# ethz-asl/multipoint

Measured on AMD Instinct MI355X. Metric: image-pairs/sec (detect+desc+match) @ 480x640, higher is better.
Workload: dtype f32

## Files before the change

multipoint_amd/csrc/api.hip:

```cpp
#include "host.h"

using namespace mp_host;

namespace {

bool debug_switch(const char* key, int* value = nullptr, int dflt = 1)
{
    const char* e = getenv("MP_DEBUG");
    if (!e) return false;
    const size_t kl = std::strlen(key);
    for (const char* q = e; *q;) {
        while (*q == ',' || *q == ' ') ++q;
        const char* end = q;
        while (*end && *end != ',') ++end;
        if ((size_t)(end - q) >= kl && std::strncmp(q, key, kl) == 0 && (q[kl] == '=' || q + kl == end || q[kl] == ' ')) {
            if (value) *value = q[kl] == '=' ? atoi(q + kl + 1) : dflt;
            return true;
        }
        q = end;
    }
    return false;
}

int kfd_num_xcc(const char* bus_id)
// ... 7 lines not shown
        FILE* f = fopen(path, "r");
        if (!f) { if (node > 8) break; else continue; }
        char key[64]; unsigned long long val = 0, loc = ~0ull, domain = 0, xcc = 0, simd = 0;
        while (fscanf(f, "%63s %llu", key, &val) == 2) {
            if (!strcmp(key, "location_id")) loc = val;
            else if (!strcmp(key, "domain")) domain = val;
            else if (!strcmp(key, "num_xcc")) xcc = val;
            else if (!strcmp(key, "simd_count")) simd = val;
        }
        fclose(f);
        if (simd > 0 && loc == want && domain == dom) return (int)xcc;
    }
    return 0;
}

}

extern "C" {

const char* mp_version(void) { return "multipoint_hip 0.1 (gfx950)"; }

const char* mp_last_error(const mp_handle* h) { return h ? h->err.c_str() : g_create_error.c_str(); }

int mp_device_shape(const mp_handle* h, int* compute_units, int* xcds, int* persistent_workgroups)
{
    if (!h) return MP_EINVAL;
    if (compute_units) *compute_units = h->ncu;
    if (xcds) *xcds = 1 << h->xcd_shift;
    if (persistent_workgroups) *persistent_workgroups = (int)persistent_grid(1ll << 40, h->ncu, h->xcd_shift);
    return MP_OK;
}

int mp_create(mp_handle** out, int device)
{
    mp_handle* h = nullptr;
    if (!out) return fail(h, MP_EINVAL, "mp_create: out is NULL");
    *out = nullptr;
    int ndev = 0;
    MP_HIP(hipGetDeviceCount(&ndev));
    if (device < 0 || device >= ndev)
        return fail(h, MP_EINVAL, "mp_create: device " + std::to_string(device) + " not available (" +
                                      std::to_string(ndev) + " HIP devices visible)");
    MP_HIP(hipSetDevice(device));
    {
        static const char* const legacy[] = {"MP_NO_WINOGRAD", "MP_WINO43", "MP_WINO43_GEN", "MP_NO_FUSE", "MP_NO_FUSE43", "MP_NO_HEAD_FUSE",
            "MP_NO_PLANAR", "MP_PLANAR", "MP_NO_PERSIST", "MP_PERSIST_MIN_ITEMS", "MP_SPLITK_MAX", "MP_F16_NO_RES", "MP_F16_NO_FUSE1",
            "MP_F16_RES_GROUPS", "MP_NCU", "MP_NXCD", "MP_POST_OVERLAP", "MP_NO_VIN", "MP_NO_POOL_FIRST"};
        static bool warned = false;
        for (const char* k : legacy)
            if (!warned && getenv(k)) {
                warned = true;
                fprintf(stderr, "libmultipoint_hip: the environment variable %s is no longer read (nor are the other MP_* kernel switches): "
                                "use MP_DEBUG=key[=value],... -- the keys are listed in csrc/api.hip (debug_switch)\n", k);
            }
    }
    hipDeviceProp_t prop;
    MP_HIP(hipGetDeviceProperties(&prop, device));
    if (std::strncmp(prop.gcnArchName, "gfx950", 6) != 0)
        return fail(h, MP_EINVAL, std::string("mp_create: kernels are built for gfx950 only, device is ") +
                                      prop.gcnArchName);
    int ncu = prop.multiProcessorCount, nxcd = 0;
    {
        char bus[64] = {0};
        if (hipDeviceGetPCIBusId(bus, sizeof bus, device) == hipSuccess) nxcd = kfd_num_xcc(bus);
        if (nxcd <= 0) nxcd = ncu >= 32 ? ncu / 32 : 1;
        int v = 0;
        if (debug_switch("ncu", &v) && v > 0 && v <= ncu) ncu = v;
        if (debug_switch("nxcd", &v) && v > 0) nxcd = v;
    }
    if (ncu < 1 || nxcd < 1 || (nxcd & (nxcd - 1)) != 0 || nxcd > ncu)
        return fail(h, MP_EINVAL, "mp_create: unsupported machine shape: " + std::to_string(ncu) + " compute units in " +
                                      std::to_string(nxcd) + " XCDs (the XCD count must be a power of two <= the CU count)");
    int xcd_shift = 0;
    while ((1 << xcd_shift) < nxcd) ++xcd_shift;
    DebugSwitches d;
    int v = 0;
    d.winograd = !debug_switch("no_winograd");
    if (debug_switch("wino43", &v) && v == 0) d.wino43 = false;
    if (debug_switch("wino43_gen", &v) && v >= 0 && v <= 2) d.wino43_gen = v;
    d.fuse_first = !debug_switch("no_fuse");
    d.fuse43 = !debug_switch("no_fuse43");
    d.head_fuse = !debug_switch("no_head_fuse");
    d.vin = !debug_switch("no_vin");
    d.planar = !debug_switch("no_planar");
    d.xplanar = d.planar && !debug_switch("no_xplanar");
    if (debug_switch("persist_min_items", &v) && v > 0) d.persist = v;
    if (debug_switch("no_persist")) d.persist = 0;
    if (debug_switch("splitk_max", &v) && v >= 1 && v <= 8) d.splitk_max = v;
    d.f16_res = !debug_switch("f16_no_res");
    d.f16_fuse1 = !debug_switch("f16_no_fuse1");
    if (debug_switch("f16_res_groups", &v) && v == 2) d.f16_res_groups = 2;
    mp_handle* hh = new mp_handle(device, ncu, xcd_shift, d);
    if (hipHostMalloc(reinterpret_cast<void**>(&hh->pinned), 4096) != hipSuccess) {
        delete hh;
        return fail(h, MP_ENOMEM, "mp_create: hipHostMalloc failed");
    }
    *out = hh;
    return MP_OK;
}

void mp_destroy(mp_handle* h)
{
    if (!h) return;
    (void)hipSetDevice(h->device);
    int* pinned = h->pinned;
    const std::vector<ProfEntry> events = std::move(h->prof_entries);
    delete h;
    if (pinned) (void)hipHostFree(pinned);
    for (auto& e : events) { (void)hipEventDestroy(e.a); (void)hipEventDestroy(e.b); }
}

int mp_profile_enable(mp_handle* h, int enable)
{
    if (!h) return MP_EINVAL;
    h->prof = enable != 0;
    h->prof_used = 0;
    return MP_OK;
}

int mp_profile_read(mp_handle* h, const char** names, float* ms, double* flop, int capacity, int* n)
{
    if (!h || !n) return MP_EINVAL;
    *n = 0;
    for (size_t i = 0; i < h->prof_used && (int)i < capacity; ++i) {
        ProfEntry& e = h->prof_entries[i];
        MP_HIP(hipEventSynchronize(e.b));
        float t = 0.f;
        MP_HIP(hipEventElapsedTime(&t, e.a, e.b));
        if (names) names[i] = e.name;
        if (ms) ms[i] = t;
        if (flop) flop[i] = e.flop;
        ++*n;
    }
    h->prof_used = 0;
    return MP_OK;
}

}
```

multipoint_amd/csrc/conv_wino43.hip:

```cpp
#include "mp_common.h"
#include "mp_device.h"
#include "mp_tile.h"

#include <algorithm>
#include <type_traits>

MP_TIMING_TABLE(g_timing_q, 256 * 8, mp_debug_read_timing_wino43)
MP_TIMING_HEIGHT(g_timing_q_sel, 480, mp_debug_select_height_wino43)

namespace {

constexpr int NPIX = 18 * 34;
constexpr int UC4 = 4;
constexpr int VB4 = UC4 * 32 * 36;
constexpr int UB4 = UC4 * 64 * 36;
constexpr int NRB = (NPIX + 63) / 64;
constexpr int RB4 = NRB * 64 * 4;
constexpr int SW4 = 8 * 36 * 2;


template <int LEAD = 0>
__device__ __forceinline__ void dma16(const float* sbase, unsigned voff_bytes, unsigned lds_byte)
{
    lds_dma<4, LEAD, 0>(sbase, voff_bytes, lds_byte);
}

template <bool POOL, bool BNF, int TC4, bool F1, bool SPLIT = false, bool VIN = false>
__global__ __launch_bounds__(512, 2) void conv_wino43_kernel(const ConvParams p)
{
    static_assert(!(F1 && SPLIT), "the fused first block is never split");
    static_assert(!(VIN && (F1 || SPLIT)), "pre-transformed input: plain launches only");
    constexpr int TR4 = 32 / TC4;
    constexpr int OY = 4 * TR4, OX = 4 * TC4;
    constexpr int PY = OY + 2, PX = OX + 2;
    static_assert(PY * PX == NPIX, "item shape");
    __shared__ __attribute__((aligned(16))) float Vs[(VIN ? 4 : 2) * VB4];
    __shared__ __attribute__((aligned(16))) float Us[2 * UB4];
    __shared__ __attribute__((aligned(16))) float raw[VIN ? 256 : 3 * RB4 + 256];
    __shared__ __attribute__((aligned(16))) float scr[VIN ? 4 : 8 * SW4];
    __shared__ __attribute__((aligned(16))) float prm[(POOL && !SPLIT ? 6 : 3) * 64];

    const int tid = threadIdx.x;
    const int lane = tid & 63;
    const int wave = __builtin_amdgcn_readfirstlane(tid >> 6);
    const int tb = wave & 1, cb = wave >> 1;
    const int NC = SPLIT ? (p.cin / UC4) >> p.ks_shift : p.cin / UC4;

    const XcdRange xr = xcd_range(p.nitems, p.xcd_shift);
    const int stride = xr.stride, item_end = xr.item_end;
    int item = xr.item;
    if (item >= item_end) return;

    struct Where { int slice, img, y0, x0, tile; const float* in_base; };
    auto decode = [&](int it) __attribute__((always_inline)) -> Where {
        Where w{};
        const int tile = (int)udiv((unsigned)it, p.magic_slices, (unsigned)p.nslices);
        w.slice = it - tile * p.nslices;
        w.tile = tile;
        const int trow = (int)udiv((unsigned)tile, p.magic_tx, (unsigned)p.tiles_x);
        const int tx = tile - trow * p.tiles_x;
        const int bi = (int)udiv((unsigned)trow, p.magic_ty, (unsigned)p.tiles_y);
        const int ty = trow - bi * p.tiles_y;
        w.img = p.img_list ? p.img_list[bi] : bi;
        w.y0 = ty * OY; w.x0 = tx * OX;
        w.in_base = p.in_planar ? p.in + (long long)w.img * (p.cin / 4) * p.H * p.W * 4
                                : p.in + (long long)w.img * p.H * p.W * p.in_cstride + p.in_coff;
        if constexpr (SPLIT)
            w.in_base += (long long)((w.slice & ((1 << p.ks_shift) - 1)) * NC) * (p.in_planar ? (long long)p.H * p.W * 4 : UC4);
        return w;
    };

    const int pix_stride = p.in_planar ? 4 : p.in_cstride;
    const long long unit_stride = p.in_planar ? (long long)p.H * p.W * 4 : UC4;
    const int x_shift = p.in_planar == MP_LAYOUT_XPLANAR ? 2 : 0, x_mask = p.in_planar == MP_LAYOUT_XPLANAR ? 3 : 0;
    const int row_stride = p.W * pix_stride;
    auto pixel_off = [&](int y, int x) __attribute__((always_inline)) -> int {
        return y * row_stride + (x >> x_shift) * pix_stride + (x & x_mask) * p.W;
    };
    unsigned rvoff[2];
    bool roff_rel = false;
    auto raw_offsets = [&](const Where& w) __attribute__((always_inline)) -> const float* {
        const bool interior = (w.y0 >= 1) && (w.y0 + OY < p.H) && (w.x0 >= 1) && (w.x0 + OX < p.W);
        if (interior) {
            if (!roff_rel) {
#pragma unroll
                for (int j = 0; j < 2; ++j) {
                    const int f = (wave + 8 * j) * 64 + lane;
                    const int py = f / PX, px = f - py * PX;
                    rvoff[j] = (f < NPIX) ? (unsigned)pixel_off(py, px + x_mask) * 4u : 0u;
                }
                roff_rel = true;
            }
            return w.in_base + pixel_off(w.y0 - 1, w.x0 - 1 - x_mask);
        }
        roff_rel = false;
#pragma unroll
        for (int j = 0; j < 2; ++j) {
            const int f = (wave + 8 * j) * 64 + lane;
            const int py = f / PX, px = f - py * PX;
            unsigned off = 0;
            if (f < NPIX) {
                const int gy = reflect_clamp(w.y0 + py - 1, p.H), gx = reflect_clamp(w.x0 + px - 1, p.W);
                off = (unsigned)pixel_off(gy, gx) * 4u;
            }
            rvoff[j] = off;
        }
        return w.in_base;
    };
    const unsigned raw_lds = lds_addr(raw), us_lds = lds_addr(Us);
    const unsigned raw_m0 = raw_lds + (unsigned)wave * 1024u;
    const unsigned raw_dummy = raw_lds + 3u * RB4 * 4u;
    auto raw_dma = [&](const float* src, unsigned boff_bytes, int j) __attribute__((always_inline)) {
        const unsigned dst = j == 0 ? raw_m0 + boff_bytes : (wave + 8 < NRB ? raw_m0 + 8192u + boff_bytes : raw_dummy);
        dma16(src, rvoff[j], dst);
    };
    const int u_cnt = wave < 4 ? 5 : 4, u_first = wave < 4 ? 5 * wave : 20 + 4 * (wave - 4);
    auto u_dma_site = [&](const float* ub, int buf, int site) __attribute__((always_inline)) {
        if constexpr (VIN) {
#pragma unroll
            for (int i = 3 * site; i < (site ? 5 : 3); ++i) {
                int b = wave + 8 * i;
                b = b < 36 ? b : 35;
                dma16(ub + b * 256, (unsigned)lane * 16u, us_lds + (unsigned)(buf * UB4 + b * 256) * 4u);
            }
            return;
        }
#pragma unroll
        for (int k = 3 * site; k < 3 * site + 3; ++k)
            if (k < u_cnt) {
                const int b = u_first + k;
                dma16<1>(ub + b * 256, (unsigned)lane * 16u, us_lds + (unsigned)(buf * UB4 + b * 256) * 4u);
            }
    };
    auto u_ptr = [&](int slice) __attribute__((always_inline)) -> const float* {
        return p.wpack + (long long)slice * NC * UB4;
    };
    auto load_prm = [&](int vslice) __attribute__((always_inline)) {
        const int slice = SPLIT ? vslice >> p.ks_shift : vslice;
        if (tid < 64) {
            int t = tid;
            if constexpr (F1) asm volatile("" : "+v"(t));
// ... 327 lines not shown
                    acc[s] = __builtin_amdgcn_mfma_f32_16x16x4f32(af[g % 3][e], bf[g % 3][e], FIRST ? zero4 : acc[s], 0, 0, 0);
                    __builtin_amdgcn_sched_barrier(0);
                    if constexpr (!VIN) { if (e != 2) tf_at(g, e, vb); }
                    if constexpr (F1) prod_at(g, e, vb);
                    if (e == 0) {
                        af[(g + 2) % 3] = *reinterpret_cast<const f32x4*>(g + 2 < 9 ? &ur[4 * (g + 2)] : &urn[4 * (g - 7)]);
                        bf[(g + 2) % 3] = *reinterpret_cast<const f32x4*>(g + 2 < 9 ? &vr[4 * (g + 2)] : &vrn[4 * (g - 7)]);
                    } else if (e == 1) {
                        if (g == 7) u_dma_site(un2, vb, 0);
                        else if (g == 8) u_dma_site(un2, vb, 1);
                        else if (g == 0) { if constexpr (VIN) v_dma(vcur, (vs + 3) & 3, 0); else if constexpr (!F1) raw_dma(rsrc, rd_byte, 0); }
                        else if (g == 1) { if constexpr (VIN) v_dma(vcur, (vs + 3) & 3, 1); else if constexpr (!F1) raw_dma(rsrc, rd_byte, 1); }
                        else if (g == 2) { if constexpr (VIN) v_dma(vcur, (vs + 3) & 3, 2); }
                    } else if (e == 2) {
                        if constexpr (!VIN) tf_at(g, 2, vb);
                    } else {
                        if (g == 6) {
#ifdef MP_TIMING
                            t_b0 = __builtin_amdgcn_s_memtime();
#endif
                            if constexpr (F1) asm volatile("s_waitcnt vmcnt(0) lgkmcnt(0)" ::: "memory");
                            else if constexpr (VIN) asm volatile("s_waitcnt vmcnt(3) lgkmcnt(0)" ::: "memory");
                            else asm volatile("s_waitcnt vmcnt(2) lgkmcnt(0)" ::: "memory");
#ifdef MP_TIMING
                            t_b1 = __builtin_amdgcn_s_memtime();
#endif
                            __syncthreads();
#ifdef MP_TIMING
                            tsum[4] += __builtin_amdgcn_s_memtime() - t_b1;
#endif
                        }
                    }
                    __builtin_amdgcn_sched_barrier(0);
                }
            }
            MP_CLOCK(t_u1);
            MP_CLOCK_ADD(0, t_u0, t_u1);
            MP_CLOCK_ADD(1, t_b0, t_b1);
        };
        auto unit = [&](const int c, auto first_tag, auto vb_tag, auto vs_tag) __attribute__((always_inline)) {
            unit_body(c, first_tag, vb_tag, vs_tag);
            if constexpr (VIN) {
                v_advance();
            } else if constexpr (F1) {
                prod_advance();
            } else {
                ld_advance();
                const unsigned ro = 3u * RB4 * 4u - rd_byte - rt_byte;
                rd_byte = rt_byte; rt_byte = ro;
            }
        };
        using VB0 = std::integral_constant<int, 0>;
        using VB1 = std::integral_constant<int, 1>;
        using VS2 = std::integral_constant<int, 2>;
        using VS3 = std::integral_constant<int, 3>;
        if constexpr (VIN) {
            unit(0, std::true_type{}, VB0{}, VB0{});
            for (int c = 1; c + 3 < NC; c += 4) {
                unit(c, std::false_type{}, VB1{}, VB1{});
                unit(c + 1, std::false_type{}, VB0{}, VS2{});
                unit(c + 2, std::false_type{}, VB1{}, VS3{});
                unit(c + 3, std::false_type{}, VB0{}, VB0{});
            }
            unit(NC - 3, std::false_type{}, VB1{}, VB1{});
            unit(NC - 2, std::false_type{}, VB0{}, VS2{});
            unit(NC - 1, std::false_type{}, VB1{}, VS3{});
        } else {
        unit(0, std::true_type{}, VB0{}, VB0{});
        for (int c = 1; c + 1 < NC; c += 2) {
            unit(c, std::false_type{}, VB1{}, VB1{});
            unit(c + 1, std::false_type{}, VB0{}, VB0{});
        }
        unit(NC - 1, std::false_type{}, VB1{}, VB1{});
        }

        MP_CLOCK(t_e0);
        MP_CLOCK_ADD(3, t_item, t_e0);
        if constexpr (F1) { if (item_next + stride < item_end) patch_dma(decode(item_next + stride), cur_par); }
        const int tl = tb * 16 + (lane & 15);
        const int cl = cb * 16 + 4 * (lane >> 4);
        const f32x4 b4 = *reinterpret_cast<const f32x4*>(&prm[cl]);
        const f32x4 s4 = *reinterpret_cast<const f32x4*>(&prm[64 + cl]);
        const f32x4 t4 = *reinterpret_cast<const f32x4*>(&prm[128 + cl]);
        const int oy = cur.y0 + 4 * (tl / TC4), ox = cur.x0 + 4 * (tl % TC4);
        const int ch0 = (SPLIT ? cur.slice >> p.ks_shift : cur.slice) * 64 + cl;
        const int cs = p.out_cstride;
        constexpr int NO = POOL ? 2 : 4;
        f32x2 keep[NO][NO];
        if constexpr (SPLIT) {
            unsigned long long* const part = reinterpret_cast<unsigned long long*>(p.split_scratch) + (long long)item * (2 * 16 * 512) + tid;
#pragma unroll
            for (int h = 0; h < 2; ++h) {
                f32x2 tcol[4][6];
#pragma unroll
                for (int j = 0; j < 6; ++j) {
                    f32x2 m[6], y[4];
#pragma unroll
                    for (int i = 0; i < 6; ++i) m[i] = f32x2{acc[6 * i + j][2 * h], acc[6 * i + j][2 * h + 1]};
                    at6s(m, y);
#pragma unroll
                    for (int a = 0; a < 4; ++a) tcol[a][j] = y[a];
                }
#pragma unroll
                for (int a = 0; a < 4; ++a) {
                    f32x2 y[4];
                    at6s(tcol[a], y);
#pragma unroll
                    for (int b = 0; b < 4; ++b)
                        part[(h * 16 + a * 4 + b) * 512] = __builtin_bit_cast(unsigned long long, y[b]);
                }
            }
        }
        if constexpr (!SPLIT) {
#pragma unroll
        for (int h = 0; h < 2; ++h) {
            f32x2 tcol[4][6];
            if constexpr (!SPLIT) {
#pragma unroll
            for (int j = 0; j < 6; ++j) {
                f32x2 m[6], y[4];
#pragma unroll
                for (int i = 0; i < 6; ++i) m[i] = f32x2{acc[6 * i + j][2 * h], acc[6 * i + j][2 * h + 1]};
                at6s(m, y);
#pragma unroll
                for (int a = 0; a < 4; ++a) tcol[a][j] = y[a];
            }
            }
            const f32x2 bb = {b4[2 * h], b4[2 * h + 1]}, ss = {s4[2 * h], s4[2 * h + 1]}, tt = {t4[2 * h], t4[2 * h + 1]};
            f32x2 res[NO][NO];
            if constexpr (POOL) {
                const f32x4 g4 = *reinterpret_cast<const f32x4*>(&prm[192 + cl]);
                const f32x4 lo4 = *reinterpret_cast<const f32x4*>(&prm[256 + cl]), hi4 = *reinterpret_cast<const f32x4*>(&prm[320 + cl]);
                const f32x2 gg = {g4[2 * h], g4[2 * h + 1]};
                const f32x2 gb = bb * gg;
                constexpr float A1 = (float)MP_W43_A, A2 = A1 * A1, A3 = A2 * A1, A4 = A2 * A2;
                const f32x2 gk[5] = {gg, gg * f32x2{A1, A1}, gg * f32x2{A2, A2}, gg * f32x2{A3, A3}, gg * f32x2{A4, A4}};
                f32x2 xv[4][4];
#pragma unroll
                for (int a = 0; a < 4; ++a) {
                    f32x2 y[4];
                    at6s(tcol[a], y);
#pragma unroll
                    for (int b = 0; b < 4; ++b) {
                        const int e = (a == 1 ? 1 : a == 2 ? 2 : 0) + (b == 1 ? 1 : b == 2 ? 2 : 0);
                        xv[a][b] = __builtin_elementwise_fma(y[b], gk[e], gb);
                    }
                }
#pragma unroll
                for (int a = 0; a < NO; ++a)
#pragma unroll
                    for (int b = 0; b < NO; ++b) {
                        f32x2 m;
#pragma unroll
                        for (int r = 0; r < 2; ++r)
                            m[r] = fmaxf(fmaxf(xv[2 * a][2 * b][r], xv[2 * a][2 * b + 1][r]), fmaxf(xv[2 * a + 1][2 * b][r], xv[2 * a + 1][2 * b + 1][r]));
                        if (BNF) {
                            m = __builtin_elementwise_fma(m, ss, tt);
                            m = f32x2{relu_bits(m[0]), relu_bits(m[1])};
                        } else {
#pragma unroll
                            for (int r = 0; r < 2; ++r)
                                asm("v_med3_i32 %0, %1, %2, %3" : "=v"(m[r]) : "v"(m[r]), "v"(lo4[2 * h + r]), "v"(hi4[2 * h + r]));
                            m = __builtin_elementwise_fma(m, ss, tt);
                        }
                        res[a][b] = m;
                    }
            } else {
            f32x2 yv[4][4];
#pragma unroll
            for (int a = 0; a < 4; ++a) {
                f32x2 y[4];
                at6s(tcol[a], y);
#pragma unroll
                for (int b = 0; b < 4; ++b) {
                    f32x2 v = w43_add_bias(y[b], a, b, bb);
                    if (BNF) { v = v * ss + tt; v = f32x2{relu_bits(v[0]), relu_bits(v[1])}; }
                    else { v = f32x2{relu_bits(v[0]), relu_bits(v[1])}; v = v * ss + tt; }
                    yv[a][b] = v;
                }
            }
#pragma unroll
            for (int a = 0; a < NO; ++a)
#pragma unroll
                for (int b = 0; b < NO; ++b) res[a][b] = yv[a][b];
            }
            if (h == 0) {
#pragma unroll
                for (int a = 0; a < NO; ++a)
#pragma unroll
                    for (int b = 0; b < NO; ++b) keep[a][b] = res[a][b];
            } else {
                const int Ho = POOL ? p.H >> 1 : p.H, Wo = POOL ? p.W >> 1 : p.W;
                const int py0 = POOL ? oy >> 1 : oy, px0 = POOL ? ox >> 1 : ox;
                const bool xpl = !POOL && p.out_planar == MP_LAYOUT_XPLANAR;
                char* const img_base = reinterpret_cast<char*>(
                    p.out_planar ? p.out + (long long)cur.img * (p.cout / 4) * Ho * Wo * 4
                                 : p.out + (long long)cur.img * Ho * Wo * cs + p.out_coff);
                const unsigned ps = xpl ? (unsigned)Wo * 4u : p.out_planar ? 16u : (unsigned)cs * 4u;
                const unsigned rs = p.out_planar ? (unsigned)Wo * 16u : (unsigned)Wo * ps;
                const unsigned o0 = xpl ? (unsigned)(((ch0 >> 2) * Ho + py0) * Wo * 4 + px0) * 4u
                                  : p.out_planar ? (unsigned)(((ch0 >> 2) * Ho + py0) * Wo + px0) * 16u
                                                 : (unsigned)((py0 * Wo + px0) * cs + ch0) * 4u;
                if (oy < p.H && ox < p.W && ch0 < p.cout) {
#pragma unroll
                    for (int a = 0; a < NO; ++a)
#pragma unroll
                        for (int b = 0; b < NO; ++b) {
                            const f32x4 v = {keep[a][b][0], keep[a][b][1], res[a][b][0], res[a][b][1]};
                            *reinterpret_cast<f32x4*>(img_base + (o0 + (unsigned)a * rs + (unsigned)b * ps)) = v;
                        }
                }
            }
        }
        }
        MP_CLOCK(t_e1);
        MP_CLOCK_ADD(2, t_e0, t_e1);
#ifdef MP_TIMING
        tsum[7] += 1;
        if (!has_next && tid == 0 && t_on)
            for (int i = 0; i < 8; ++i) g_timing_q[blockIdx.x * 8 + i] = tsum[i];
#endif
        if (!has_next) { dma_wait(); return; }
        if (next_slice != cur.slice) {
            __syncthreads();
            load_prm(next_slice);
        }
        item = item_next;
        cur = decode(item);
        cur_par ^= 1;
        up = unext;
    }
}

template <int TC4>
__global__ __launch_bounds__(256) void wino43_vprod_kernel(const ConvParams p, long long ntb)
{
    constexpr int TR4 = 32 / TC4, OY = 4 * TR4, OX = 4 * TC4;
    __shared__ __attribute__((aligned(16))) float st[19456];
    const int ncp = p.cin >> 1, NC = p.cin / UC4;
    const int TL = 256 / ncp;
    const int RS = TL * 36 + 4;
    const int groups = 32 / TL;
    const int tid = threadIdx.x;
    const int cp = tid % ncp, tlc = tid / ncp;
    const long long tb = (long long)blockIdx.x / groups;
    const int t0 = ((int)((long long)blockIdx.x % groups)) * TL, t = t0 + tlc;
    (void)ntb;
    const int tx = (int)(tb % p.tiles_x);
    const long long trow = tb / p.tiles_x;
    const int ty = (int)(trow % p.tiles_y);
    const int bi = (int)(trow / p.tiles_y);
    const int img = p.img_list ? p.img_list[bi] : bi;
    const int wy = ty * OY + 4 * (t / TC4) - 1, wx = tx * OX + 4 * (t % TC4) - 1;
    const float* const base = p.in + (long long)img * p.H * p.W * p.in_cstride + p.in_coff + 2 * cp;
    int gx[6];
#pragma unroll
    for (int j = 0; j < 6; ++j) gx[j] = reflect_clamp(wx + j, p.W);
    f32x2 r[6][6];
#pragma unroll
    for (int j = 0; j < 6; ++j) {
        f32x2 d[6], o[6];
#pragma unroll
        for (int i = 0; i < 6; ++i)
            d[i] = *reinterpret_cast<const f32x2*>(base + ((long long)reflect_clamp(wy + i, p.H) * p.W + gx[j]) * p.in_cstride);
        bt6(d, o);
#pragma unroll
        for (int i = 0; i < 6; ++i) r[i][j] = o[i];
    }
    float* const dst0 = st + (2 * cp) * RS + tlc * 36;
    float* const dst1 = dst0 + RS;
#pragma unroll
    for (int i = 0; i < 6; i += 2) {
        f32x2 a[6], b[6];
        bt6(r[i], a);
        bt6(r[i + 1], b);
        *reinterpret_cast<f32x4*>(dst0 + 6 * i) = f32x4{a[0][0], a[1][0], a[2][0], a[3][0]};
        *reinterpret_cast<f32x4*>(dst0 + 6 * i + 4) = f32x4{a[4][0], a[5][0], b[0][0], b[1][0]};
        *reinterpret_cast<f32x4*>(dst0 + 6 * i + 8) = f32x4{b[2][0], b[3][0], b[4][0], b[5][0]};
        *reinterpret_cast<f32x4*>(dst1 + 6 * i) = f32x4{a[0][1], a[1][1], a[2][1], a[3][1]};
        *reinterpret_cast<f32x4*>(dst1 + 6 * i + 4) = f32x4{a[4][1], a[5][1], b[0][1], b[1][1]};
        *reinterpret_cast<f32x4*>(dst1 + 6 * i + 8) = f32x4{b[2][1], b[3][1], b[4][1], b[5][1]};
    }
    __syncthreads();
    const int q4 = TL * 9, total4 = p.cin * q4;
    float* const gbase = p.vglobal + (tb * NC * 4 * 32 + t0) * 36;
    for (int i = tid; i < total4; i += 256) {
        const int row = i / q4, w = i - row * q4;
        *reinterpret_cast<f32x4*>(gbase + (long long)row * (32 * 36) + w * 4) = *reinterpret_cast<const f32x4*>(st + row * RS + w * 4);
    }
}

template <bool POOL, int TC4, bool F1 = false, bool SPLIT = false>
int launch_q(const ConvParams& p, hipStream_t s)
{
    constexpr int OY = 4 * (32 / TC4), OX = 4 * TC4;
    ConvParams q = p;
    if (SPLIT) q.nslices = p.nslices << p.ks_shift;
    q.tiles_x = (p.W + OX - 1) / OX; q.tiles_y = (p.H + OY - 1) / OY;
    const long long nitems = (long long)p.B * q.tiles_x * q.tiles_y * q.nslices;
    if (nitems <= 0) return 0;
    if (tile_items(q, nitems)) return 1;
    const unsigned grid = persistent_grid(nitems, p.ncu, p.xcd_shift);
    const ConvParams& pp = q;
    if (p.bn_first) hipLaunchKernelGGL((conv_wino43_kernel<POOL, true, TC4, F1, SPLIT>), dim3(grid), dim3(512), 0, s, pp);
    else hipLaunchKernelGGL((conv_wino43_kernel<POOL, false, TC4, F1, SPLIT>), dim3(grid), dim3(512), 0, s, pp);
    return 0;
}

template <int TC4>
int launch_vin(const ConvParams& p, hipStream_t s)
{
    constexpr int OY = 4 * (32 / TC4), OX = 4 * TC4;
    ConvParams q = p;
    q.tiles_x = (p.W + OX - 1) / OX; q.tiles_y = (p.H + OY - 1) / OY;
    const long long ntb = (long long)p.B * q.tiles_x * q.tiles_y, nitems = ntb * q.nslices;
    if (nitems <= 0) return 0;
    if (tile_items(q, nitems)) return 1;
    const ConvParams& pp = q;
    const int tl = 256 / (p.cin / 2);
    hipLaunchKernelGGL((wino43_vprod_kernel<TC4>), dim3((unsigned)(ntb * (32 / tl))), dim3(256), 0, s, pp, ntb);
    const unsigned grid = persistent_grid(nitems, p.ncu, p.xcd_shift);
    if (p.bn_first) hipLaunchKernelGGL((conv_wino43_kernel<false, true, TC4, false, false, true>), dim3(grid), dim3(512), 0, s, pp);
    else hipLaunchKernelGGL((conv_wino43_kernel<false, false, TC4, false, false, true>), dim3(grid), dim3(512), 0, s, pp);
    return 0;
}

template <bool POOL, bool SPLIT = false>
int launch_shape(const ConvParams& p, hipStream_t s)
{
    const long long wide = (long long)((p.W + 31) / 32) * ((p.H + 15) / 16), tall = (long long)((p.W + 15) / 16) * ((p.H + 31) / 32);
    return tall < wide ? launch_q<POOL, 4, false, SPLIT>(p, s) : launch_q<POOL, 8, false, SPLIT>(p, s);
}

}

bool conv_wino43_supports(const ConvParams& p)
{
    return !p.pad_zero && p.cin % 8 == 0 && p.cout % 4 == 0 && p.H % 4 == 0 && p.W % 4 == 0 && p.H >= 4 && p.W >= 4 &&
           p.in_cstride % 4 == 0 && p.in_coff % 4 == 0 && p.out_cstride % 4 == 0 && p.out_coff % 4 == 0;
}

long long conv_wino43_vglobal_floats(const ConvParams& p)
{
    const long long wide = (long long)((p.W + 31) / 32) * ((p.H + 15) / 16), tall = (long long)((p.W + 15) / 16) * ((p.H + 31) / 32);
    return (long long)p.B * std::min(wide, tall) * (p.cin / UC4) * VB4;
}

long long conv_wino43_items(const ConvParams& p)
{
    const long long wide = (long long)((p.W + 31) / 32) * ((p.H + 15) / 16), tall = (long long)((p.W + 15) / 16) * ((p.H + 31) / 32);
    return (long long)p.B * std::min(wide, tall) * p.nslices;
}

int launch_conv_wino43(const ConvParams& p, bool pool, hipStream_t s, bool fuse_first)
{
    if (p.out_planar == MP_LAYOUT_XPLANAR && pool) return 2;
    if ((p.in_planar == MP_LAYOUT_XPLANAR || p.out_planar == MP_LAYOUT_XPLANAR) && p.ks_shift > 0) return 2;
    if (fuse_first) return pool && p.cin == 64 ? launch_q<true, 8, true>(p, s) : 2;
    if (p.vglobal) {
        if (pool || p.ks_shift > 0 || p.cin % 16 != 0 || p.in_planar || p.cin > 256 || 256 % (p.cin / 2) != 0 || (p.cin / 2) < 8) return 2;
        const long long wide = (long long)((p.W + 31) / 32) * ((p.H + 15) / 16), tall = (long long)((p.W + 15) / 16) * ((p.H + 31) / 32);
        return tall < wide ? launch_vin<4>(p, s) : launch_vin<8>(p, s);
    }
    if (p.ks_shift > 0) {
        const int ncs = (p.cin / 4) >> p.ks_shift;
        if (ncs < 4 || (ncs & 1) || (ncs << p.ks_shift) * 4 != p.cin || !p.split_scratch) return 2;
        const int rc = pool ? launch_shape<true, true>(p, s) : launch_shape<false, true>(p, s);
        return rc ? rc : launch_split_reduce(p, 1, pool, s);
    }
    return pool ? launch_shape<true>(p, s) : launch_shape<false>(p, s);
}
```

multipoint_amd/csrc/forward.hip:

```cpp
#include "host.h"

using namespace mp_host;

namespace {

int pick_mbw(int H, int W)
{
    long long best = -1;
    int arg = 32;
    for (int mbw : {32, 16, 8}) {
        const int tw = mbw, th = 256 / mbw;
        const long long area = (long long)((H + th - 1) / th) * th * ((W + tw - 1) / tw) * tw;
        if (best < 0 || area < best) { best = area; arg = mbw; }
    }
    return arg;
}

void prof_begin(mp_handle* h, const char* name, double flop, hipStream_t s)
{
    if (!h->prof) return;
    if (h->prof_used == h->prof_entries.size()) {
        ProfEntry e{};
        (void)hipEventCreate(&e.a); (void)hipEventCreate(&e.b);
        h->prof_entries.push_back(e);
// ... 76 lines not shown
    EncoderPlan P;
    if (h->cfg.mixed_precision) {
        const ConvLayer& L0 = E.conv[0];
        P.conv[0].fuse_first = h->dbg.f16_res && h->dbg.f16_fuse1 && h->cfg.reflection_pad && !E.first_pool && L0.pool &&
                               L0.cin == 64 && L0.cout == 64 && L0.nslices == 1;
        for (int i = 0; i < E.nconv; ++i) P.conv[i].kernel = f16_kind(h, E.conv[i], E.conv[i].cin, 0, P.conv[i].fuse_first);
        return P;
    }
    for (int i = 0, hh = E.first_pool ? H / 2 : H, ww = E.first_pool ? W / 2 : W; i < E.nconv; ++i) {
        const ConvLayer& L = E.conv[i];
        ConvLaunch& c = P.conv[i];
        c.kernel = wino43_kind(h, L, hh, ww, L.cin, 0, L.cout, 0);
        if (i == 0) {
            const bool fuse43 = c.kernel == Kernel::wino43 && h->dbg.fuse43 && L.pool && L.cin == 64 && L.cout == 64 &&
                                h->cfg.channel_version == 0 && L.u43pack_f1;
            c.fuse_first = h->dbg.fuse_first && h->cfg.channel_version == 0 && !E.first_pool && (h->policy.direct || fuse43);
        }
        const bool producer = i == 0 ? !E.first_pool : P.conv[i - 1].kernel != Kernel::direct && E.conv[i - 1].pool;
        c.in_planar = h->dbg.planar && c.kernel != Kernel::direct && producer ? MP_LAYOUT_PLANAR : MP_LAYOUT_NHWC;
        plan_split_vin(h, L, nb, hh, ww, fwd_batch, c);
        if (i > 0 && h->dbg.xplanar && !E.conv[i - 1].pool && P.conv[i - 1].kernel == Kernel::wino43 && P.conv[i - 1].ks_shift == 0 &&
            c.kernel == Kernel::wino43 && c.ks_shift == 0 && !c.vin)
            c.in_planar = MP_LAYOUT_XPLANAR;
        if (i > 0) P.conv[i - 1].out_planar = c.in_planar;
        if (L.pool) { hh /= 2; ww /= 2; }
    }
    return P;
}


template <typename P, typename T>
int conv_geometry(const mp_handle* h, const ConvLayer& L, P& p, const T* in, int in_cstride, int in_coff, T* out, int out_cstride,
                  int out_coff, int B, int H, int W)
{
    p.in = in; p.out = out; p.B = B; p.H = H; p.W = W;
    p.in_cstride = in_cstride; p.in_coff = in_coff; p.cin = L.cin;
    p.out_cstride = out_cstride; p.out_coff = out_coff; p.cout = L.cout; p.nslices = L.nslices;
    p.pad_zero = h->cfg.reflection_pad ? 0 : 1; p.bn_first = h->cfg.bn_first;
    p.ncu = h->ncu; p.xcd_shift = h->xcd_shift;
    const int mbw = L.taps == 9 ? pick_mbw(H, W) : 32, th = 256 / mbw;
    if (L.taps == 9) { p.tiles_x = (W + mbw - 1) / mbw; p.tiles_y = (H + th - 1) / th; }
    else p.total_px = (long long)B * H * W;
    return mbw;
}

template <typename P, typename T>
void conv1_geometry(const mp_handle* h, P& c1, const float* images, T* out, int B, int H, int W)
{
    c1.in = images; c1.out = out; c1.B = B; c1.H = H; c1.W = W;
    c1.pad_zero = h->cfg.reflection_pad ? 0 : 1; c1.bn_first = h->cfg.bn_first;
}

template <typename T>
int run_conv(mp_handle* h, const ConvLayer& L, const ConvLaunch& c, const T* in, int in_cstride, int in_coff, T* out,
             int out_cstride, int out_coff, int B, int H, int W, const int* img_list, hipStream_t s,
             const FirstLayer* first = nullptr, const float* images = nullptr)
{
    constexpr bool f16 = std::is_same<T, _Float16>::value;
    typename std::conditional<f16, ConvParamsH, ConvParams>::type p{};
    const int mbw = conv_geometry(h, L, p, in, in_cstride, in_coff, out, out_cstride, out_coff, B, H, W);
    p.scale = L.scale; p.shift = L.shift; p.img_list = img_list;
    if (c.fuse_first) {
        p.img = images; p.w1 = f16 ? first->w_h : first->w; p.b1 = f16 ? first->bias_h : first->bias;
        p.s1 = first->scale; p.t1 = first->shift;
    }
    if constexpr (f16) {
        p.wpack = L.wpack_h; p.bias = L.bias_h;
        p.dummy = static_cast<_Float16*>(h->f16_dummy.p);
        p.res_groups = h->dbg.f16_res_groups;
    } else {
        p.wpack = c.kernel == Kernel::direct ? L.wpack : L.u43pack; p.bias = L.bias;
        p.relu = L.relu ? 1 : 0;
        p.persist = h->dbg.persist;
        p.in_planar = c.in_planar; p.out_planar = c.out_planar;
        if (c.fuse_first && c.kernel != Kernel::direct) {
            p.wpack = L.u43pack_f1; p.bias = L.bias_f1; p.w1 = first->w_f1; p.b1 = first->bias_f1; p.s1 = nullptr; p.t1 = nullptr;
        }
        if (c.ks_shift) {
            const int rc = ensure(h, h->split_ws, (size_t)(conv_wino43_items(p) << c.ks_shift) * (2 * 16 * 512 * 8));
            if (rc) return rc;
            p.ks_shift = c.ks_shift; p.split_scratch = static_cast<float*>(h->split_ws.p);
        }
        if (c.vin) {
            if (ensure(h, h->vin_ws, (size_t)conv_wino43_vglobal_floats(p) * 4) == MP_OK) p.vglobal = static_cast<float*>(h->vin_ws.p);
            else { (void)hipGetLastError(); h->err.clear(); }
        }
    }
    prof_begin(h, c.fuse_first ? "enc.conv1+2" : L.name,
               2.0 * L.taps * L.cin * L.cout * (double)B * H * W + (c.fuse_first ? 2.0 * 9 * 64 * (double)B * H * W : 0.0), s);
    int big = 0;
    if constexpr (f16) {
        if (c.kernel == Kernel::f16_res) {
            big = launch_conv_f16_res(p, mbw, L.pool, s);
        } else if (c.kernel == Kernel::f16_res_slices) {
            for (int sl = 0; sl < L.nslices && !big; ++sl) {
                ConvParamsH q = p;
                q.wpack = p.wpack + (size_t)sl * 36 * 2 * 64 * 8;
                q.bias = p.bias + 64 * sl; q.scale = p.scale + 64 * sl; q.shift = p.shift + 64 * sl;
                q.out_coff = out_coff + 64 * sl; q.cout = 64; q.nslices = 1;
                big = conv_f16_res_supports(q, L.taps) ? launch_conv_f16_res(q, mbw, L.pool, s) : 2;
            }
        } else {
            big = launch_conv_f16(p, L.taps, mbw, L.pool, s);
        }
    } else {
        big = c.kernel == Kernel::wino43b ? launch_conv_wino43b(p, L.pool, s)
            : c.kernel == Kernel::wino43  ? launch_conv_wino43(p, L.pool, s, c.fuse_first)
                                          : launch_conv_mfma(p, L.taps, mbw, L.pool, c.fuse_first, s);
    }
    prof_end(h, s);
    return big ? launch_failed(h, big, L.name, B, H, W) : MP_OK;
}

template <typename T>
void run_first(mp_handle* h, const Encoder& E, bool out_planar, const float* images, T* out, int B, int H, int W,
               const int* img_list, hipStream_t s)
{
    constexpr bool f16 = std::is_same<T, _Float16>::value;
    typename std::conditional<f16, Conv1ParamsH, Conv1Params>::type c1{};
    conv1_geometry(h, c1, images, out, B, H, W);
    c1.w = f16 ? E.first.w_h : E.first.w; c1.bias = f16 ? E.first.bias_h : E.first.bias;
    c1.scale = E.first.scale; c1.shift = E.first.shift; c1.img_list = img_list;
    c1.pool = E.first_pool ? 1 : 0;
    prof_begin(h, "enc.conv1", 2.0 * 9 * 64 * (double)B * H * W, s);
    if constexpr (f16) {
        launch_conv_first_f16(c1, s);
    } else {
        c1.channels = E.first.channels; c1.out_planar = out_planar ? 1 : 0;
        launch_conv_first(c1, s);
    }
    prof_end(h, s);
}

struct FwdWorkspace { size_t P, Q, Lg, X, R, lists, bytes; };
FwdWorkspace fwd_workspace(bool f16, int B, int H, int W)
{
    const size_t el = f16 ? 2 : 4, px = (size_t)B * H * W, npx = px / 64;
    FwdWorkspace w{};
    w.Q = w.P + px * 64 * el;
    w.Lg = w.Q + px * 16 * el;
    w.X = w.Lg + npx * (f16 ? 128 : 80) * el;
    w.R = w.X + npx * 128 * el;
    w.lists = w.R + (f16 ? npx * 256 * el : 0);
    w.bytes = w.lists + 2 * 1024 * 4 + 256;
    return w;
}

struct ImageRoute {
    int counts[2] = {0, 0};
    std::vector<int> ids;
};

ImageRoute route_images(const mp_handle* h, const unsigned char* is_optical, int B)
{
    ImageRoute r;
    if (!h->cfg.multispectral) { r.counts[0] = B; return r; }
    r.ids.assign(1024, 0);
    for (int b = 0; b < B; ++b) {
        if (is_optical[b]) r.ids[512 + r.counts[1]++] = b;
        else r.ids[r.counts[0]++] = b;
    }
    return r;
}

template <typename T>
int run_forward(mp_handle* h, const float* images, const ImageRoute& route, int B, int H, int W, float* prob, float* logits, float* desc,
                hipStream_t s)
{
// ... 327 lines not shown
```

multipoint_amd/csrc/host.h:

```cpp
#pragma once
#include "../../include/multipoint_hip.h"
#include "mp_common.h"

#include <cmath>
#include <cstdio>
#include <cstdlib>
#include <cstring>
#include <map>
#include <string>
#include <type_traits>
#include <vector>

namespace mp_host {

inline std::string g_create_error;

struct DevBuf {
    void* p = nullptr;
    size_t bytes = 0;
    DevBuf(void* p_ = nullptr, size_t bytes_ = 0) : p(p_), bytes(bytes_) {}
    DevBuf(DevBuf&& o) noexcept : p(o.p), bytes(o.bytes) { o.p = nullptr; o.bytes = 0; }
    ~DevBuf() { if (p) (void)hipFree(p); }
};

struct ConvLayer {
    const char* name = "";
    float *wpack = nullptr, *bias = nullptr, *scale = nullptr, *shift = nullptr;
    float* u43pack = nullptr;
    float *u43pack_f1 = nullptr, *bias_f1 = nullptr;
    _Float16* wpack_h = nullptr;
    float* bias_h = nullptr;
    int cin = 0, cout = 0, taps = 9, nslices = 0;
    bool pool = false, relu = true;
};

struct FirstLayer {
    int channels = 64;
    float *w = nullptr, *bias = nullptr, *scale = nullptr, *shift = nullptr;
    float *w_h = nullptr, *bias_h = nullptr;
    float *w_f1 = nullptr, *bias_f1 = nullptr;
};

struct Encoder {
    FirstLayer first;
    ConvLayer conv[7];
    int nconv = 7;
    bool first_pool = false;
};

struct BnLayer {
    std::string name;
    int channels = 0;
    float *gamma = nullptr, *beta = nullptr;
    long long offset = 0;
};

struct ProfEntry {
    const char* name;
    hipEvent_t a, b;
    double flop;
};

struct DebugSwitches {
    bool winograd = true, wino43 = true, fuse_first = true, fuse43 = true, head_fuse = true, vin = true, planar = true;
    bool xplanar = true, f16_res = true, f16_fuse1 = true;
    int wino43_gen = 0, persist = 8, splitk_max = 8, f16_res_groups = 3;
};

struct ConvPolicy {
    bool direct = false;
    bool wino43 = true;
    int wino43_gen = 0;
    int splitk_max = 8;
};

struct MiRefine {
    void* workspace = nullptr;
    MiLaunch L{};
    int P = 0, normalized = 0;
    double sigma = 0.0;
    long long smooth_stride = 0;
    unsigned* counts = nullptr;
    float* warped = nullptr;
    double *smooth_a = nullptr, *smooth_b = nullptr, *cand = nullptr, *values = nullptr;
    const double* reg_init = nullptr;
    MiNmState* state = nullptr;
    int* nact = nullptr;
};

}

struct mp_handle {
    mp_handle(int device_, int ncu_, int xcd_shift_, const mp_host::DebugSwitches& dbg_)
        : device(device_), ncu(ncu_), xcd_shift(xcd_shift_), dbg(dbg_) {}
    const int device;
    const int ncu, xcd_shift;
    const mp_host::DebugSwitches dbg;
    std::string err;
    bool loaded = false;
    mp_model_config cfg{};
    mp_host::ConvPolicy policy;
    std::vector<mp_host::DevBuf> weights;
    mp_host::Encoder enc[2];
    mp_host::ConvLayer heads3, det1, desc1;
    mp_host::DevBuf fwd_ws;
    mp_host::DevBuf nms_ws;
    mp_host::DevBuf match_ws;
    mp_host::DevBuf metrics_ws;
    mp_host::DevBuf split_ws;
    mp_host::DevBuf vin_ws;
    mp_host::DevBuf bs_ws;
    std::vector<mp_host::BnLayer> bn_layers;
    float* bn_ident = nullptr;
    mp_host::DevBuf nms_state;
    mp_host::DevBuf kp_scratch;
    mp_host::DevBuf nms_total;
    int last_nms_rounds = 0;
    mp_host::DevBuf tie_state;
    float tie_eps = 6e-5f;
    int tie_min = 4;
    int tie_last_B = 0;
    mp_host::DevBuf tie_pairs;
    int tie_pairs_min = 16;
    int head_channels = 256;
    mp_host::DevBuf f16_dummy;
    int* pinned = nullptr;
    mp_host::MiRefine mi;
    std::map<int, mp_host::DevBuf> fft_tw;
    mp_host::DevBuf draw_ws;
    std::vector<mp_host::DevBuf> draw_retired;
    bool prof = false;
    bool head_fallback_noted = false;
    std::vector<mp_host::ProfEntry> prof_entries;
    size_t prof_used = 0;
};

namespace mp_host {

inline int fail(mp_handle* h, int code, const std::string& msg)
{
    if (h) h->err = msg; else g_create_error = msg;
    return code;
}

#define MP_HIP(expr)                                                                          \
    do {                                                                                      \
        hipError_t _e = (expr);                                                               \
        if (_e != hipSuccess)                                                                 \
// ... 32 lines not shown
```

multipoint_amd/csrc/mp_common.h:

```cpp
#pragma once
#include <hip/hip_runtime.h>
#include <stdint.h>

typedef float f32x16 __attribute__((ext_vector_type(16)));
typedef float f32x4 __attribute__((ext_vector_type(4)));
typedef float f32x2 __attribute__((ext_vector_type(2)));

#define MP_WAVE 64

enum { MP_LAYOUT_NHWC = 0, MP_LAYOUT_PLANAR = 1, MP_LAYOUT_XPLANAR = 2 };

struct ConvParams {
    const float* in;
    float* out;
    const float* wpack;
    const float* bias;
    const float* scale;
    const float* shift;
    const int* img_list;
    const float* img;
    const float *w1, *b1, *s1, *t1;
    int B, H, W;
    int in_cstride, in_coff, cin;
    int out_cstride, out_coff, cout;
    int nslices;
    int tiles_x, tiles_y;
    int pad_zero;
    int bn_first;
    int relu;
    long long total_px;
    unsigned magic_slices, magic_tx, magic_ty;
    int nitems;
    int persist;
    int in_planar, out_planar;
    int ncu, xcd_shift;
    int ks_shift;
    float* split_scratch;
    float* vglobal;
};

struct XcdRange { int item, item_end, stride; };
__device__ __forceinline__ XcdRange xcd_range(int nitems, int xcd_shift)
{
    const int nxcd = 1 << xcd_shift;
    const int per_xcd = (nitems + nxcd - 1) >> xcd_shift;
    const int xcd = (int)blockIdx.x & (nxcd - 1);
    XcdRange r;
    r.stride = (int)gridDim.x >> xcd_shift;
    r.item_end = min((xcd + 1) * per_xcd, nitems);
    r.item = xcd * per_xcd + ((int)blockIdx.x >> xcd_shift);
    return r;
}
inline unsigned persistent_grid(long long nitems, int ncu, int xcd_shift, int per_cu = 1)
{
    const long long nxcd = 1ll << xcd_shift;
    const long long full = ((long long)ncu * per_cu) / nxcd * nxcd;
    const long long need = (nitems + nxcd - 1) / nxcd * nxcd;
    return (unsigned)(need < full ? need : full);
}

struct Conv1Params {
    const float* in;
    float* out;
    const float* w;
    const float* bias; const float* scale; const float* shift;
    const int* img_list;
    int B, H, W;
    int pad_zero, bn_first;
    int channels;
    int out_planar;
    int pool;
};

int launch_conv_mfma(const ConvParams& p, int taps, int mbw, bool pool, bool fuse1, hipStream_t s);
void launch_conv_first(const Conv1Params& p, hipStream_t s);
int launch_conv_mfma_linear(const ConvParams& p, int mbw, hipStream_t s);
void launch_conv_first_linear(const Conv1Params& p, hipStream_t s);
#ifndef MP_W43_A
#define MP_W43_A 0.75
#endif
#ifndef MP_W43_B
#define MP_W43_B 1.5
#endif
constexpr unsigned long long pk_const2(double lo, double hi)
{
    return (unsigned long long)__builtin_bit_cast(unsigned, (float)lo) | ((unsigned long long)__builtin_bit_cast(unsigned, (float)hi) << 32);
}
constexpr double W43A = MP_W43_A, W43B = MP_W43_B;
constexpr unsigned long long K_AB = pk_const2(W43A, W43B), K_BA = pk_const2(W43B, W43A), K_A2B2 = pk_const2(W43A * W43A, W43B * W43B),
                             K_B2A2 = pk_const2(W43B * W43B, W43A * W43A),
                             K_PS = pk_const2(W43A * W43A * W43B * W43B, W43A * W43A + W43B * W43B);
static_assert((double)(float)(W43A * W43A * W43B * W43B) == W43A * W43A * W43B * W43B && (double)(float)(W43A * W43A + W43B * W43B) ==
              W43A * W43A + W43B * W43B, "the transform coefficients must be exact in fp32");
template <int HI>
__device__ __forceinline__ f32x2 pk_fma_k(f32x2 a, unsigned long long k, f32x2 c)
{
    f32x2 d;
    if (HI) asm("v_pk_fma_f32 %0, %1, %2, %3 op_sel:[0,1,0] op_sel_hi:[1,1,1]" : "=v"(d) : "v"(a), "s"(k), "v"(c));
    else asm("v_pk_fma_f32 %0, %1, %2, %3 op_sel:[0,0,0] op_sel_hi:[1,0,1]" : "=v"(d) : "v"(a), "s"(k), "v"(c));
    return d;
}
template <int HI>
__device__ __forceinline__ f32x2 pk_fnma_k(f32x2 a, unsigned long long k, f32x2 c)
{
    f32x2 d;
    if (HI) asm("v_pk_fma_f32 %0, %1, %2, %3 op_sel:[0,1,0] op_sel_hi:[1,1,1] neg_lo:[1,0,0] neg_hi:[1,0,0]" : "=v"(d) : "v"(a), "s"(k), "v"(c));
    else asm("v_pk_fma_f32 %0, %1, %2, %3 op_sel:[0,0,0] op_sel_hi:[1,0,1] neg_lo:[1,0,0] neg_hi:[1,0,0]" : "=v"(d) : "v"(a), "s"(k), "v"(c));
    return d;
}
__device__ __forceinline__ void bt6(const f32x2 d[6], f32x2 r[6])
{
    const f32x2 t0 = pk_fnma_k<1>(d[2], K_A2B2, d[4]);
    const f32x2 t1 = pk_fnma_k<1>(d[1], K_A2B2, d[3]);
    const f32x2 t2 = pk_fnma_k<0>(d[2], K_A2B2, d[4]);
    const f32x2 t3 = pk_fnma_k<0>(d[1], K_A2B2, d[3]);
    r[0] = pk_fma_k<0>(d[0], K_PS, pk_fnma_k<1>(d[2], K_PS, d[4]));
    r[1] = pk_fma_k<0>(t1, K_AB, t0);
    r[2] = pk_fnma_k<0>(t1, K_AB, t0);
    r[3] = pk_fma_k<1>(t3, K_AB, t2);
    r[4] = pk_fnma_k<1>(t3, K_AB, t2);
    r[5] = pk_fma_k<0>(d[1], K_PS, pk_fnma_k<1>(d[3], K_PS, d[5]));
// ... 285 lines not shown
```

Measured before the change: 3501.

## Pack Winograd 4x3 input tiles densely across images in VIN path

Adds a dense tile numbering for the pre-transformed-input (VIN) Winograd F(4,3) path. 4x4 output tiles from all images are enumerated linearly and grouped 32 per block, instead of per-image rectangular 2D tile blocks. This is meant to remove padding waste at image edges and the per-image block rounding. The cost is extra magic-number divisions per tile, zero-fill and bounds checks for the tail block, and changed workspace sizing. It is on by default and can be disabled through a debug switch.

```diff
diff --git a/multipoint_amd/csrc/api.hip b/multipoint_amd/csrc/api.hip
--- a/multipoint_amd/csrc/api.hip
+++ b/multipoint_amd/csrc/api.hip
@@ -113,6 +113,7 @@
     d.fuse43 = !debug_switch("no_fuse43");
     d.head_fuse = !debug_switch("no_head_fuse");
     d.vin = !debug_switch("no_vin");
+    d.vin_dense = !debug_switch("no_vin_dense");
     d.planar = !debug_switch("no_planar");
     d.xplanar = d.planar && !debug_switch("no_xplanar");
     if (debug_switch("persist_min_items", &v) && v > 0) d.persist = v;
diff --git a/multipoint_amd/csrc/conv_wino43.hip b/multipoint_amd/csrc/conv_wino43.hip
--- a/multipoint_amd/csrc/conv_wino43.hip
+++ b/multipoint_amd/csrc/conv_wino43.hip
@@ -57,6 +57,7 @@
         const int tile = (int)udiv((unsigned)it, p.magic_slices, (unsigned)p.nslices);
         w.slice = it - tile * p.nslices;
         w.tile = tile;
+        if constexpr (VIN) { if (p.dense_tiles) { w.in_base = p.in; return w; } }
         const int trow = (int)udiv((unsigned)tile, p.magic_tx, (unsigned)p.tiles_x);
         const int tx = tile - trow * p.tiles_x;
         const int bi = (int)udiv((unsigned)trow, p.magic_ty, (unsigned)p.tiles_y);
@@ -550,7 +551,19 @@
         const f32x4 b4 = *reinterpret_cast<const f32x4*>(&prm[cl]);
         const f32x4 s4 = *reinterpret_cast<const f32x4*>(&prm[64 + cl]);
         const f32x4 t4 = *reinterpret_cast<const f32x4*>(&prm[128 + cl]);
-        const int oy = cur.y0 + 4 * (tl / TC4), ox = cur.x0 + 4 * (tl % TC4);
+        int oy = cur.y0 + 4 * (tl / TC4), ox = cur.x0 + 4 * (tl % TC4);
+        unsigned dimg = 0u;
+        bool live = true;
+        if constexpr (VIN) {
+            if (p.dense_tiles) {
+                const unsigned d = (unsigned)cur.tile * 32u + (unsigned)tl;
+                dimg = udiv(d, p.magic_ti, (unsigned)p.tiles_img);
+                const unsigned r = d - dimg * (unsigned)p.tiles_img;
+                const unsigned ty = udiv(r, p.magic_tw, (unsigned)p.tiles_w);
+                oy = 4 * (int)ty; ox = 4 * (int)(r - ty * (unsigned)p.tiles_w);
+                live = d < (unsigned)p.dense_tiles;
+            }
+        }
         const int ch0 = (SPLIT ? cur.slice >> p.ks_shift : cur.slice) * 64 + cl;
         const int cs = p.out_cstride;
         constexpr int NO = POOL ? 2 : 4;
@@ -666,10 +679,11 @@
                                  : p.out + (long long)cur.img * Ho * Wo * cs + p.out_coff);
                 const unsigned ps = xpl ? (unsigned)Wo * 4u : p.out_planar ? 16u : (unsigned)cs * 4u;
                 const unsigned rs = p.out_planar ? (unsigned)Wo * 16u : (unsigned)Wo * ps;
-                const unsigned o0 = xpl ? (unsigned)(((ch0 >> 2) * Ho + py0) * Wo * 4 + px0) * 4u
-                                  : p.out_planar ? (unsigned)(((ch0 >> 2) * Ho + py0) * Wo + px0) * 16u
-                                                 : (unsigned)((py0 * Wo + px0) * cs + ch0) * 4u;
-                if (oy < p.H && ox < p.W && ch0 < p.cout) {
+                unsigned o0 = xpl ? (unsigned)(((ch0 >> 2) * Ho + py0) * Wo * 4 + px0) * 4u
+                            : p.out_planar ? (unsigned)(((ch0 >> 2) * Ho + py0) * Wo + px0) * 16u
+                                           : (unsigned)((py0 * Wo + px0) * cs + ch0) * 4u;
+                if constexpr (VIN) o0 += dimg * ((unsigned)(Ho * Wo) * (unsigned)(p.out_planar ? p.cout : cs) * 4u);
+                if (oy < p.H && ox < p.W && ch0 < p.cout && live) {
 #pragma unroll
                     for (int a = 0; a < NO; ++a)
 #pragma unroll
@@ -714,12 +728,21 @@
     const long long tb = (long long)blockIdx.x / groups;
     const int t0 = ((int)((long long)blockIdx.x % groups)) * TL, t = t0 + tlc;
     (void)ntb;
-    const int tx = (int)(tb % p.tiles_x);
-    const long long trow = tb / p.tiles_x;
-    const int ty = (int)(trow % p.tiles_y);
-    const int bi = (int)(trow / p.tiles_y);
-    const int img = p.img_list ? p.img_list[bi] : bi;
-    const int wy = ty * OY + 4 * (t / TC4) - 1, wx = tx * OX + 4 * (t % TC4) - 1;
+    int img, wy, wx;
+    if (p.dense_tiles) {
+        const unsigned d = min((unsigned)tb * 32u + (unsigned)t, (unsigned)p.dense_tiles - 1u);
+        const unsigned bi = udiv(d, p.magic_ti, (unsigned)p.tiles_img), rest = d - bi * (unsigned)p.tiles_img;
+        const unsigned ty = udiv(rest, p.magic_tw, (unsigned)p.tiles_w);
+        img = (int)bi;
+        wy = 4 * (int)ty - 1; wx = 4 * (int)(rest - ty * (unsigned)p.tiles_w) - 1;
+    } else {
+        const int tx = (int)(tb % p.tiles_x);
+        const long long trow = tb / p.tiles_x;
+        const int ty = (int)(trow % p.tiles_y);
+        const int bi = (int)(trow / p.tiles_y);
+        img = p.img_list ? p.img_list[bi] : bi;
+        wy = ty * OY + 4 * (t / TC4) - 1; wx = tx * OX + 4 * (t % TC4) - 1;
+    }
     const float* const base = p.in + (long long)img * p.H * p.W * p.in_cstride + p.in_coff + 2 * cp;
     int gx[6];
 #pragma unroll
@@ -752,9 +775,11 @@
     __syncthreads();
     const int q4 = TL * 9, total4 = p.cin * q4;
     float* const gbase = p.vglobal + (tb * NC * 4 * 32 + t0) * 36;
+    const int w_end = p.dense_tiles ? 9 * (int)std::min<long long>(TL, std::max<long long>(0, p.dense_tiles - (tb * 32 + t0))) : q4;
     for (int i = tid; i < total4; i += 256) {
         const int row = i / q4, w = i - row * q4;
-        *reinterpret_cast<f32x4*>(gbase + (long long)row * (32 * 36) + w * 4) = *reinterpret_cast<const f32x4*>(st + row * RS + w * 4);
+        const f32x4 v = *reinterpret_cast<const f32x4*>(st + row * RS + w * 4);
+        *reinterpret_cast<f32x4*>(gbase + (long long)row * (32 * 36) + w * 4) = w < w_end ? v : f32x4{0.f, 0.f, 0.f, 0.f};
     }
 }
 
@@ -775,13 +800,35 @@
     return 0;
 }
 
+long long vin_dense_tiles(const ConvParams& p)
+{
+    if (!p.vin_dense || p.img_list) return 0;
+    const long long tw = p.W / 4, ti = (long long)(p.H / 4) * tw, total = (long long)p.B * ti;
+    if (total <= 0 || (total + 32) * std::max(ti, tw) >= 0x80000000ll) return 0;
+    if ((long long)p.B * p.H * p.W * std::max(p.out_cstride, p.cout) * 4 >= 0x100000000ll) return 0;
+    return total;
+}
+
+long long tile_blocks(const ConvParams& p)
+{
+    const long long wide = (long long)((p.W + 31) / 32) * ((p.H + 15) / 16), tall = (long long)((p.W + 15) / 16) * ((p.H + 31) / 32);
+    const long long dense = vin_dense_tiles(p);
+    return dense ? (dense + 31) / 32 : (long long)p.B * std::min(wide, tall);
+}
+
 template <int TC4>
 int launch_vin(const ConvParams& p, hipStream_t s)
 {
     constexpr int OY = 4 * (32 / TC4), OX = 4 * TC4;
     ConvParams q = p;
     q.tiles_x = (p.W + OX - 1) / OX; q.tiles_y = (p.H + OY - 1) / OY;
-    const long long ntb = (long long)p.B * q.tiles_x * q.tiles_y, nitems = ntb * q.nslices;
+    q.dense_tiles = (int)vin_dense_tiles(p);
+    if (q.dense_tiles) {
+        auto magic = [](int d) -> unsigned { return d <= 1 ? 0u : (unsigned)((0x100000000ull / (unsigned)d) + 1ull); };
+        q.tiles_w = p.W / 4; q.tiles_img = (p.H / 4) * q.tiles_w;
+        q.magic_ti = magic(q.tiles_img); q.magic_tw = magic(q.tiles_w);
+    }
+    const long long ntb = tile_blocks(p), nitems = ntb * q.nslices;
     if (nitems <= 0) return 0;
     if (tile_items(q, nitems)) return 1;
     const ConvParams& pp = q;
@@ -810,14 +857,12 @@
 
 long long conv_wino43_vglobal_floats(const ConvParams& p)
 {
-    const long long wide = (long long)((p.W + 31) / 32) * ((p.H + 15) / 16), tall = (long long)((p.W + 15) / 16) * ((p.H + 31) / 32);
-    return (long long)p.B * std::min(wide, tall) * (p.cin / UC4) * VB4;
+    return tile_blocks(p) * (p.cin / UC4) * VB4;
 }
 
 long long conv_wino43_items(const ConvParams& p)
 {
-    const long long wide = (long long)((p.W + 31) / 32) * ((p.H + 15) / 16), tall = (long long)((p.W + 15) / 16) * ((p.H + 31) / 32);
-    return (long long)p.B * std::min(wide, tall) * p.nslices;
+    return tile_blocks(p) * p.nslices;
 }
 
 int launch_conv_wino43(const ConvParams& p, bool pool, hipStream_t s, bool fuse_first)
diff --git a/multipoint_amd/csrc/forward.hip b/multipoint_amd/csrc/forward.hip
--- a/multipoint_amd/csrc/forward.hip
+++ b/multipoint_amd/csrc/forward.hip
@@ -182,8 +182,9 @@
             p.ks_shift = c.ks_shift; p.split_scratch = static_cast<float*>(h->split_ws.p);
         }
         if (c.vin) {
+            p.vin_dense = h->dbg.vin_dense ? 1 : 0;
             if (ensure(h, h->vin_ws, (size_t)conv_wino43_vglobal_floats(p) * 4) == MP_OK) p.vglobal = static_cast<float*>(h->vin_ws.p);
-            else { (void)hipGetLastError(); h->err.clear(); }
+            else { (void)hipGetLastError(); h->err.clear(); p.vin_dense = 0; }
         }
     }
     prof_begin(h, c.fuse_first ? "enc.conv1+2" : L.name,
diff --git a/multipoint_amd/csrc/host.h b/multipoint_amd/csrc/host.h
--- a/multipoint_amd/csrc/host.h
+++ b/multipoint_amd/csrc/host.h
@@ -63,7 +63,7 @@
 
 struct DebugSwitches {
     bool winograd = true, wino43 = true, fuse_first = true, fuse43 = true, head_fuse = true, vin = true, planar = true;
-    bool xplanar = true, f16_res = true, f16_fuse1 = true;
+    bool xplanar = true, f16_res = true, f16_fuse1 = true, vin_dense = true;
     int wino43_gen = 0, persist = 8, splitk_max = 8, f16_res_groups = 3;
 };
 
diff --git a/multipoint_amd/csrc/mp_common.h b/multipoint_amd/csrc/mp_common.h
--- a/multipoint_amd/csrc/mp_common.h
+++ b/multipoint_amd/csrc/mp_common.h
@@ -37,6 +37,9 @@
     int ks_shift;
     float* split_scratch;
     float* vglobal;
+    int vin_dense;
+    int dense_tiles, tiles_img, tiles_w;
+    unsigned magic_ti, magic_tw;
 };
 
 struct XcdRange { int item, item_end, stride; };
```

Result: no change. 3511 (median of 6 runs) (+0.3%).
